# shionhonda/IaGo

Measured on AMD Instinct MI355X. Metric: self-play games/sec, higher is better.
Workload: dtype f16 MFMA operands (float32 split in 2 / 3 pieces), f32 accumulate; u64 bitboards; f32 / f64 tree statistics

## Files before the change

iago_amd/_lib.py:

```python
import ctypes as C
import os

HERE = os.path.dirname(os.path.abspath(__file__))
SO_PATH = os.environ.get("IAGO_HIP_LIB") or os.path.join(HERE, "libiago_hip.so")

IAGO_OK = 0
IAGO_ERR_INVALID, IAGO_ERR_HIP, IAGO_ERR_CAPACITY = -1, -2, -3
IAGO_MAX_TURNS = 128
IAGO_ROLLOUT_TABLE_FLOATS = 3 * 2 * 256 * 8 + 64 + 4 + 2 * 512
ROLLOUT_MODE_INDEX = 3 * 2 * 256 * 8 + 64
TRACE_PASS = 0xFF

SYMBOLS = [
    "iago_abi_version", "iago_last_error", "iago_device_count",
    "iago_legal_moves", "iago_apply_moves", "iago_play_turn", "iago_encode_planes", "iago_encode_planes_indexed",
    "iago_judge", "iago_sample_moves", "iago_augment8",
    "iago_rollout_build_table", "iago_rollout",
    "iago_policy_forward_split3", "iago_value_forward_split", "iago_value_rollout",
    "iago_mcts_reset", "iago_leaf_values", "iago_mcts_best_move", "iago_mcts_advance_root", "iago_mcts_compact",
    "iago_mcts_mix_backup_lookahead", "iago_mcts_store_priors", "iago_mcts_descend",
    "iago_mcts_search_persistent", "iago_mcts_search_capacity", "iago_mcts_search_streams_create",
    "iago_mcts_search_streams_destroy", "iago_mcts_search_split", "iago_selfplay_policy",
    "iago_policy_grad_workspace_bytes", "iago_policy_reinforce_grad", "iago_adam_chainer",
]
# ... 144 lines not shown

class MctsLookahead(C.Structure):
    _fields_ = [
        ("trigger", C.c_int32), ("slots", C.c_int32), ("next_seq", C.c_void_p), ("cache_seq", C.c_void_p),
        ("cache", C.c_void_p), ("q_count", C.c_void_p), ("q_capacity", C.c_int32), ("path_stride", C.c_int32),
        ("q_own", C.c_void_p), ("q_opp", C.c_void_p), ("q_game", C.c_void_p), ("q_seq", C.c_void_p),
        ("error", C.c_void_p), ("clear_word", C.c_void_p), ("path", C.c_void_p), ("path_len", C.c_void_p),
        ("z_log", C.c_void_p), ("z_log_n", C.c_void_p), ("z_log_rows", C.c_int32), ("reserved", C.c_int32),
        ("async_", C.c_void_p), ("value_ahead", C.c_void_p),
    ]


class MctsValueAhead(C.Structure):
    _fields_ = [
        ("x_capacity", C.c_int32), ("row_capacity", C.c_int32), ("x_count", C.c_void_p),
        ("x_game", C.c_void_p), ("x_node", C.c_void_p), ("x_own", C.c_void_p), ("x_opp", C.c_void_p),
        ("row_count", C.c_void_p), ("row_own", C.c_void_p), ("row_opp", C.c_void_p), ("row_node", C.c_void_p),
        ("row_v", C.c_void_p), ("total", C.c_void_p),
    ]


SEARCH_QUEUE_ENTRIES = 4096
SEARCH_GAMES_PER_WORKGROUP = 32
MATCH_MCTS_COLOUR_1 = 2
MATCH_MCTS_COLOUR_2 = 3
MATCH_KEY = 0x4D415443
MATCH_SEED_XOR = MATCH_KEY << 32
EXPLORE_KEY = 0x4558504C
EXPLORE_SEED_XOR = EXPLORE_KEY << 32
CAP_KEY = 0x43415050
CAP_SEED_XOR = CAP_KEY << 32
CTL_BAD_DRAW = 13
REC_DRAWN = 2
REC_FAST = 4


class MctsSearchArgs(C.Structure):
    _fields_ = [
        ("tree", C.c_void_p), ("root_own", C.c_void_p), ("root_opp", C.c_void_p), ("active", C.c_void_p),
        ("c_puct", C.c_float), ("lmbda", C.c_float), ("n_thr", C.c_int32), ("n_sims", C.c_int32),
        ("net_workgroups", C.c_int32), ("time_limit_ms", C.c_int32),
        ("value", C.c_void_p), ("policy", C.c_void_p), ("rollout", C.c_void_p),
        ("cur_node", C.c_void_p), ("cur_own", C.c_void_p), ("cur_opp", C.c_void_p), ("path", C.c_void_p),
        ("path_stride", C.c_int32), ("z_log_rows", C.c_int32), ("done", C.c_void_p), ("roll", C.c_void_p),
        ("leaf_value", C.c_void_p), ("z_log", C.c_void_p), ("z_log_n", C.c_void_p), ("q_slots", C.c_void_p),
        ("ctl", C.c_void_p), ("rep_v", C.c_void_p), ("rep_p", C.c_void_p), ("totals", C.c_void_p),
# ... 203 lines not shown
```

iago_amd/csrc/search_kernel.hip:

```cpp
#include "mcts_dev.hpp"
#include "conv_trunk_body.hpp"
#include "conv_policy_body.hpp"
#include "sample_dev.hpp"
#include "../../include/iago_hip_serving.h"

#include <cstdlib>
#include <string>
#include <vector>

namespace {
using namespace iago;
using namespace iago_mcts;

typedef unsigned long long u64;
#define RLX_AGENT __ATOMIC_RELAXED, __HIP_MEMORY_SCOPE_AGENT

constexpr uint32_t QCAP = IAGO_SEARCH_QUEUE_ENTRIES;
constexpr int CTL_FINISHED = 2, CTL_ABORT = 3;
__host__ __device__ constexpr int ctl_head(uint32_t q) { return 8 + 2 * (int)q; }
__host__ __device__ constexpr int ctl_tail(uint32_t q) { return 9 + 2 * (int)q; }
enum { ST_READY = 0, ST_WAIT_PRIOR, ST_PRIOR_READY, ST_ROLL, ST_ROLL_FRESH, ST_WAIT_VALUE, ST_HAVE_VALUE, ST_DONE, ST_TURN, ST_MOVE,
       ST_WAIT_DRAW, ST_DRAW,
       ST_IDLE };
constexpr int CTL_NO_CHILDREN = 4;
// ... 43 lines not shown
    int8_t *rec_move;
    int32_t *rec_pi;
    int32_t games_total, stream;
    u64 *vtable;
    uint32_t vtable_mask;
    int64_t *trace;
    int32_t trace_rows;
    int32_t policy_xcds;
    int32_t pair_backlog;
    int32_t pace_margin, pace_backlog;
    int32_t ahead_idle;
    int32_t roll_defer;
    int32_t path_lds_cap;
    int32_t wave;
    float vloss;
    int64_t n_slots;
    int64_t *wave_timing;
    int32_t park_empties;
    uint8_t *parked;
    int32_t *park_stones;
    uint8_t *park_pass;
    int32_t explore_turns;
    int32_t cap_fast, cap_full_256;
};

__device__ __forceinline__ u64 ld(const u64 *p) { return __hip_atomic_load(p, RLX_AGENT); }
__device__ __forceinline__ void st(u64 *p, u64 x) { __hip_atomic_store(p, x, RLX_AGENT); }

__device__ __forceinline__ void send_request(const SearchParams &S, uint32_t kind, int64_t g, uint32_t reply_tag,
                                             uint64_t own, uint64_t opp)
{
    const uint32_t t = __hip_atomic_fetch_add(&S.ctl[ctl_tail(kind)], 1u, RLX_AGENT);
    u64 *e = S.q_slots + ((u64)kind * QCAP + t % QCAP) * 8u;
    const u64 tag = (u64)(t + 1u) << 32;
    st(e + 1, tag | reply_tag);
    st(e + 2, tag | (uint32_t)own);
    st(e + 3, tag | (uint32_t)(own >> 32));
    st(e + 4, tag | (uint32_t)opp);
    st(e + 5, tag | (uint32_t)(opp >> 32));
    st(e + 0, tag | (kind << 31) | (uint32_t)g);
    atomicAdd((unsigned long long *)&S.totals[(uint32_t)g == NOBODY ? 11 : kind], 1ull);
}

__device__ __forceinline__ uint32_t vtable_slot(const SearchParams &S, uint64_t own, uint64_t opp)
{
    uint64_t h = own * 0x9E3779B97F4A7C15ull ^ (opp + 0xD1B54A32D192ED03ull) * 0xBF58476D1CE4E5B9ull;
// ... 128 lines not shown
struct Game {
    int state;
    uint32_t epoch;
    int n_done, turn, stones;
    bool pass_flg, g_over;
    uint64_t g_own, g_opp;
};

struct Cursor {
    int node, fc, k, nv, nvv;
    uint32_t vbits;
    uint64_t own, opp;
    int path_n, leaf;
    bool may_expand, leaf_fresh;
    float v_reply;
};

struct GameLds {
    uint64_t h_own[GAMES_PER_WG], h_opp[GAMES_PER_WG];
    int32_t h_stream[GAMES_PER_WG];
    int32_t h_game[GAMES_PER_WG];
    int32_t h_budget[GAMES_PER_WG];
    uint8_t h_fast[GAMES_PER_WG];
    uint32_t wg_count[6];
    int32_t roll_list[GAMES_PER_WG];
    uint32_t roll_wave[BLOCK / 64], roll_wave_old[BLOCK / 64];
    int32_t pace[4];
    uint32_t claimed;
    int8_t h_z[GAMES_PER_WG];
};
template <bool WAVE> struct GameShared : GameLds {};
template <> struct GameShared<true> : GameLds {
    int32_t wv_next[GAMES_PER_WG], wv_size[GAMES_PER_WG], wv_block[GAMES_PER_WG];
    long long wv_time[4];
};

template <bool WAVE>
__device__ __forceinline__ Slot make_slot(const SearchParams &S, const int wg)
{
    Slot I;
    I.wg = wg;
    I.tid = threadIdx.x;
    I.gl = I.tid >> 3;
    I.L = make_lane8(threadIdx.x);
    I.r = I.L.l8;
    I.mine = I.tid < 8 * S.games_per_wg;
    I.g = (int64_t)wg * S.games_per_wg + I.gl;
// ... 157 lines not shown
        }
        G.state = ST_DONE;
        if (S.trace && I.r == 0u && I.g < S.trace_rows) {
            int64_t *row = S.trace + 4 * ((int64_t)S.trace_rows - 1 - I.g);
            row[0] = wall_clock64() - t0;
            row[1] = G.epoch;
            row[2] = G.turn;
        }
    } else {
        G.state = ST_TURN;
    }
}

template <bool PARK>
__device__ __forceinline__ void turn_boundary(const SearchParams &S, const iago_row::HwParams &R, const Slot &I, GameLds &sh,
                                              Game &G, const Cursor &C, bool &busy, const long long t0)
{
    const Tree &T = S.T;
    for (int rep = 0; rep < 6; rep++) {
        const bool at_move = G.state == ST_MOVE, at_turn = G.state == ST_TURN, at_draw = G.state == ST_DRAW;
        if (__builtin_amdgcn_ballot_w64(at_move || at_turn || at_draw) == 0ull)
            break;
        busy = busy || at_move || at_turn || at_draw;
        const bool explores = S.explore_turns > 0 && at_move && G.turn < S.explore_turns;
        const bool caps = S.cap_fast > 0 && at_turn;
        uint32_t w = 0u;
        if (__builtin_amdgcn_ballot_w64(explores || caps) != 0ull)
            w = turn_word(R.key0, R.key1 ^ (caps ? CAP_KEY : EXPLORE_KEY), R.id_base + (uint32_t)sh.h_game[I.gl], (uint32_t)G.turn);
        if (caps) {
            const bool fast = cap_fast_turn(w, (uint32_t)S.cap_full_256);
            sh.h_budget[I.gl] = fast ? S.cap_fast : S.n_sims;
            sh.h_fast[I.gl] = fast ? 1 : 0;
        }
        const uint64_t lg = group8_legal(to_lane(G.g_own, I.L), to_lane(G.g_opp, I.L), I.L);
        const bool can_move = lg != 0ull && !G.g_over;
        const int code = (at_turn && can_move && !S.stream) ? (int)S.active[I.g] : 0;
        const bool match = code == 2 || code == 3;
        const bool forced = match && G.stones > 62 && __popcll(lg) == 1;
        const bool policy_turn = match && !forced && (G.turn & 1) == (code == 2 ? 1 : 0);
        if (policy_turn) {
            G.epoch++;
            if (I.r == 0u)
                send_request(S, KIND_POLICY, I.g, G.epoch, G.g_own, G.g_opp);
            G.state = ST_WAIT_DRAW;
        }
        bool park = false;
// ... 54 lines not shown
        send_request(S, KIND_POLICY, I.g, G.epoch, C.own, C.opp);
    G.state = ST_WAIT_PRIOR;
    if (sh.pace[3] > 0 && I.need_v) {
        uint64_t rest = group8_legal(to_lane(C.own, I.L), to_lane(C.opp, I.L), I.L);
        while (rest) {
            const int a2 = (int)__builtin_ctzll(rest);
            rest &= rest - 1ull;
            uint64_t c_own = C.own, c_opp = C.opp;
            place_stone(c_own, c_opp, a2, I.L);
            uint32_t known = 0u, by = 0u;
            if (I.r == 0u && !vtable_get(S, c_own, c_opp, known, by) && atomicSub(&sh.pace[3], 1) > 0)
                send_request(S, KIND_VALUE, (int64_t)NOBODY, (uint32_t)I.g, c_own, c_opp);
        }
    }
}

template <bool WAVE>
__device__ __forceinline__ void reach_leaf(const SearchParams &S, const Slot &I, GameShared<WAVE> &sh, Game &G, Cursor &C,
                                           bool descending)
{
    if (descending && C.fc >= 0 && I.r == 0u)
        S.T.overflow[I.gt] = 1;
    C.leaf = C.node;
    const float c = __uint_as_float(C.vbits);
    C.leaf_fresh = I.need_v && c != c;
    bool ask = C.leaf_fresh;
    if (S.vtable_mask) {
        uint32_t hit = 0u, bits = 0u, by = 0u;
        if (C.leaf_fresh && I.r == 0u && vtable_get(S, C.own, C.opp, bits, by)) {
            hit = 1u;
            atomicAdd((unsigned long long *)&S.totals[8], 1ull);
            if (by == (uint32_t)I.g)
                atomicAdd((unsigned long long *)&S.totals[12], 1ull);
        }
        hit = group8_add(hit);
        bits = group8_add(I.r == 0u ? bits : 0u);
        if (hit) {
            C.vbits = bits;
            ask = false;
        }
    }
    if (ask)
        G.epoch++;
    if (I.r == 0u) {
        S.cur_node[I.g] = C.node;
        S.cur_own[I.g] = C.own;
// ... 26 lines not shown
    if (grow) {
        const int kn = lg ? __popcll(lg) : 1;
        if (lg != 0ull && kn > 1 && !have_priors) {
            need_prior = true;
            descending = false;
        } else {
            C.may_expand = false;
            const uint32_t fc1 = alloc_children(T, I.gt, kn, I.r == 0u);
            if (fc1 != 0u) {
                const int nf = (int)fc1 - 1;
                make_children(T, I.base, nf, C.node, lg, I.r,
                              [&](int a) { return __uint_as_float((uint32_t)ld(&S.rep_p[I.g * 64 + a])); });
                if (I.r == 0u)
                    link_children(T, I.base + C.node, nf, kn);
                C.fc = nf;
                C.k = kn;
            }
        }
    }
    __threadfence_block();
}

template <bool WAVE>
__device__ __forceinline__ void select_child(const SearchParams &S, const Slot &I, Cursor &C, bool descending)
{
    const int kk = descending ? C.k : 0;
    const double sq = sqrt((double)(WAVE ? C.nv + C.nvv : C.nv));
    double best_v = -INFINITY;
    int best_i = 0x7fffffff;
    uint32_t pl[4] = {0u, 0u, 0u, 0u};
    for (int j0 = (int)I.r; j0 < kk; j0 += 16) {
        const int j1 = j0 + 8;
        const bool two = j1 < kk;
        const int64_t c0 = I.base + C.fc + j0, c1 = two ? I.base + C.fc + j1 : c0;
        uint4 s0, l0, s1, l1;
        node_record(S.T, c0, s0, l0);
        node_record(S.T, c1, s1, l1);
        score_child<WAVE>(S.c_puct, (double)S.vloss, s0, l0, j0, sq, best_v, best_i, pl);
        if (two)
            score_child<WAVE>(S.c_puct, (double)S.vloss, s1, l1, j1, sq, best_v, best_i, pl);
    }
    argmax_step_payload<DPP_XOR1>(best_v, best_i, pl);
    argmax_step_payload<DPP_XOR2>(best_v, best_i, pl);
    argmax_step_payload<DPP_HALF_MIRROR>(best_v, best_i, pl);
    uint64_t own = C.own, opp = C.opp;
    place_stone(own, opp, descending ? (int)(int8_t)(pl[2] & 0xFFu) : -1, I.L);
    if (descending) {
        C.own = own;
        C.opp = opp;
        cursor_to<WAVE>(C, C.fc + best_i, pl[0], pl[1], pl[2], pl[2] >> 16, pl[3]);
    }
}

template <bool WAVE>
__device__ __forceinline__ bool descend(const SearchParams &S, const Slot &I, GameShared<WAVE> &sh, Game &G, Cursor &C,
                                        int pace_limit, int &st_levels, int &st_children)
{
    bool my_turn = true;
    if constexpr (WAVE)
        my_turn = I.s_in == sh.wv_next[I.tl];
    const bool fresh_start = G.state == ST_READY && (WAVE ? my_turn : G.turn * S.n_sims + G.n_done <= pace_limit);
    bool descending = fresh_start || (G.state == ST_PRIOR_READY && my_turn);
    bool have_priors = G.state == ST_PRIOR_READY;
    bool skip_record = G.state == ST_PRIOR_READY;
    bool need_prior = false;
    if (fresh_start) {
        const int root = S.T.root[I.gt];
        C.own = I.whole ? G.g_own : S.root_own[I.gt];
        C.opp = I.whole ? G.g_opp : S.root_opp[I.gt];
        uint4 s0, l0;
        node_record(S.T, I.base + root, s0, l0);
        cursor_to<WAVE>(C, root, l0.x, s0.x, l0.z, l0.w, s0.w);
        C.path_n = 0;
        C.may_expand = true;
    }
    const bool went = descending;
    for (int depth = 0; depth < MAX_DEPTH; depth++) {
        if (descending && !skip_record) {
            if (I.r == 0u) {
                if (C.path_n < S.path_stride) {
                    if (I.path_at >= 0)
                        ((int32_t *)iago_trunk::trunk_lds)[I.path_at + C.path_n] = C.node;
                    else
                        I.gpath[C.path_n] = C.node;
                }
                else
                    S.T.overflow[I.gt] = 1;
            }
            C.path_n++;
        }
        skip_record = false;
        expand(S, I, C, descending, have_priors, need_prior);
        have_priors = false;
        descending = descending && C.fc >= 0;
        if (__builtin_amdgcn_ballot_w64(descending) == 0ull)
            break;
        st_levels += descending ? 1 : 0;
        st_children += descending ? C.k : 0;
        if (__builtin_amdgcn_ballot_w64(descending && C.k != 1) == 0ull) {
            uint4 s0, l0;
            node_record(S.T, descending ? I.base + C.fc : I.base, s0, l0);
            const bool pass_child = (int)(int8_t)(l0.z & 0xFFu) < 0;
            if (__builtin_amdgcn_ballot_w64(descending && !pass_child) == 0ull) {
                if (descending) {
                    const uint64_t t = C.own;
                    C.own = C.opp;
                    C.opp = t;
                    cursor_to<WAVE>(C, C.fc, l0.x, s0.x, l0.z, l0.w, s0.w);
                }
                continue;
            }
        }
        select_child<WAVE>(S, I, C, descending);
    }
    if (went) {
        if (need_prior)
            ask_priors(S, I, sh, G, C);
        else
            reach_leaf<WAVE>(S, I, sh, G, C, descending);
    }
    if (I.exists && I.r == 0u)
        S.roll[I.g] = (I.need_z && (G.state == ST_ROLL || G.state == ST_ROLL_FRESH)) ? 1 : 0;
    return went;
}

struct CtlWords {
    uint32_t abort, idle, t0, h0, t1, h1, play, prog, next;
};
__device__ __forceinline__ CtlWords read_ctl(const SearchParams &S, int tid)
{
    CtlWords c = {0u, 0u, 0u, 0u, 0u, 0u, 0u, 0u, 0u};
    if (tid == 0) {
        if (S.stream)
            c.next = __hip_atomic_load(&S.ctl[CTL_NEXT_GAME], RLX_AGENT);
        c.abort = __hip_atomic_load(&S.ctl[CTL_ABORT], RLX_AGENT);
        c.idle = __hip_atomic_load(&S.ctl[CTL_IDLE], RLX_AGENT);
        c.t0 = __hip_atomic_load(&S.ctl[ctl_tail(0)], RLX_AGENT);
// ... 131 lines not shown
                limit = (int)(c.prog / c.play) + S.pace_margin;
        }
        sh.pace[2] = limit;
    }
    return stop != 0;
}

__device__ __forceinline__ bool stream_claim(const SearchParams &S, const Slot &I, GameLds &sh, Game &G, bool &in_play)
{
    const Tree &T = S.T;
    const int n_here = (int)min((int64_t)S.games_per_wg, I.n_slots - (int64_t)I.wg * S.games_per_wg);
    if (I.tid == 0)
        sh.claimed = __hip_atomic_fetch_add(&S.ctl[CTL_NEXT_GAME], (uint32_t)n_here, RLX_AGENT);
    __syncthreads();
    const int64_t next = T.n_games + (int64_t)sh.claimed + I.gl;
    if (I.exists && next < S.games_total) {
        start_game(G, S.game_own[next], S.game_opp[next]);
        if (I.r == 0u) {
            S.done[I.g] = 0;
            fresh_root(T, I.g, I.base);
            atomicAdd(&sh.pace[1], 1);
        }
        sh.h_game[I.gl] = (int32_t)next;
        G.state = ST_TURN;
        in_play = true;
    }
    return __syncthreads_and(!I.mine || G.state == ST_DONE) != 0;
}

template <bool WAVE>
__device__ __forceinline__ void epilogue(const SearchParams &S, const Slot &I, GameShared<WAVE> &sh, const Game &G,
                                         int st_levels, int st_children, const long long t0)
{
    if (I.exists && I.r == 0u && S.stats) {
        if (WAVE) {
            atomicAdd(&S.stats[2 * I.gt], st_levels);
            atomicAdd(&S.stats[2 * I.gt + 1], st_children);
        } else {
            S.stats[2 * I.g] += st_levels;
            S.stats[2 * I.g + 1] += st_children;
        }
    }
    if constexpr (WAVE) {
        if (I.tid < 4 && S.wave_timing)
            atomicAdd((unsigned long long *)&S.wave_timing[I.tid], (unsigned long long)sh.wv_time[I.tid]);
    }
    if (I.exists && I.r == 0u && G.state != ST_DONE && __hip_atomic_load(&S.ctl[CTL_ABORT], RLX_AGENT) != 0u) {
        S.cur_node[I.g] = (int32_t)G.epoch;
        S.leaf_value[I.g] = (float)G.state;
    }
    if (I.tid == 0) {
        atomicAdd((unsigned long long *)&S.totals[2], (unsigned long long)sh.wg_count[0]);
        atomicAdd((unsigned long long *)&S.totals[6], (unsigned long long)sh.wg_count[1]);
        atomicAdd((unsigned long long *)&S.totals[10], (unsigned long long)sh.wg_count[2]);
        atomicAdd((unsigned long long *)&S.totals[13], (unsigned long long)sh.wg_count[3]);
        atomicAdd((unsigned long long *)&S.totals[14], (unsigned long long)sh.wg_count[4]);
        atomicAdd((unsigned long long *)&S.totals[15], (unsigned long long)sh.wg_count[5]);
        atomicAdd((unsigned long long *)&S.totals[7], (unsigned long long)(wall_clock64() - t0));
        __hip_atomic_fetch_add(&S.ctl[CTL_FINISHED], 1u, RLX_AGENT);
    }
}

template <bool WAVE, bool PARK = false>
__device__ __forceinline__ void game_workgroup(const SearchParams &S, const iago_row::HwParams &R, const long long t0, const int wg)
{
    __shared__ GameShared<WAVE> sh;
    const Slot I = make_slot<WAVE>(S, wg);
    const bool first = I.exists && I.gt < S.games_total && (S.stream || S.active[I.gt] != 0);
    Game G;
    G.state = (first && S.n_sims > 0) ? (I.whole ? ST_TURN : ST_READY) : ST_DONE;
    G.epoch = 0u;
    if constexpr (WAVE) {
        const int m = S.n_sims < I.W ? S.n_sims : I.W;
        if (G.state == ST_READY && I.s_in >= m)
            G.state = ST_IDLE;
        if (I.tid < GAMES_PER_WG) {
            sh.wv_next[I.tid] = 0;
            sh.wv_size[I.tid] = m;
            sh.wv_block[I.tid] = 0;
        }
        if (I.tid < 4)
            sh.wv_time[I.tid] = 0;
    }
    if (I.exists && I.r == 0u) {
        S.done[I.g] = 0;
        S.roll[I.g] = 0;
    }
    if (I.mine) {
        sh.h_game[I.gl] = (int32_t)I.gt;
        sh.h_budget[I.gl] = S.n_sims;
        sh.h_fast[I.gl] = 0;
    }
    const bool whole_game = I.whole && I.exists && I.g < S.games_total;
    start_game(G, whole_game ? S.game_own[I.g] : 0ull, whole_game ? S.game_opp[I.g] : 0ull);
    if (whole_game && G.state == ST_DONE && I.r == 0u)
        S.n_turns[I.g] = 0;
    Cursor C = {};
    C.fc = -1;
    int st_levels = 0, st_children = 0;
    if (I.tid < 6)
        sh.wg_count[I.tid] = 0u;
    bool deferred = false;
    bool table_ready = false;
    int contrib = 0;
    bool in_play = G.state != ST_DONE;
    if (I.tid < 4)
        sh.pace[I.tid] = I.tid == 2 ? 0x7fffffff : 0;
    __syncthreads();
    if (I.mine && in_play && I.r == 0u)
        atomicAdd(&sh.pace[1], 1);
    int pace_limit = 0x7fffffff;

    for (;;) {
        const long long c_it = WAVE ? wall_clock64() : 0;
        bool busy = false;
        if (I.mine) {
            take_replies(S, R, I, sh, G, C);
            if (!WAVE && G.state == ST_HAVE_VALUE) {
                finish_playout(S, I, sh, G, C, true, C.v_reply);
                busy = true;
            }
            if (!WAVE && I.whole)
                turn_boundary<PARK>(S, R, I, sh, G, C, busy, t0);
// ... 357 lines not shown
    if (k == 0) {
        int n_cu = 0, per = 0;
        if (hipDeviceGetAttribute(&n_cu, hipDeviceAttributeMultiprocessorCount, dev) != hipSuccess ||
            hipOccupancyMaxActiveBlocksPerMultiprocessor(&per, (const void *)search_kernel, 256, (size_t)search_lds()) != hipSuccess)
            return iago_fail(IAGO_ERR_HIP, "iago_mcts_search_capacity: the device does not answer");
        if (n_cu < 1 || per < 1 || per > 255)
            return iago_fail(IAGO_ERR_CAPACITY, "iago_mcts_search_capacity: the search kernel does not fit a CU of this device");
        k = (int32_t)(n_cu << 8 | per);
        known[dev & 63].store(k, std::memory_order_release);
    }
    *cus = k >> 8;
    *workgroups_per_cu = k & 255;
    return IAGO_OK;
}

struct iago_search_streams {
    int device;
    int32_t cus, game_cus;
    hipStream_t game, net;
    hipEvent_t ready, game_done, net_done;
};

namespace {
int check_args(const iago_mcts_search_args *a, const iago_search_wave_args *wv)
{
    if (!a || !a->tree || !a->value || !a->policy || !a->rollout)
        return iago_fail(IAGO_ERR_INVALID, "iago_mcts_search_persistent: null args");
    const iago_mcts_tree *tree = a->tree;
    if (tree->n_games < 1 || tree->capacity < 1 || !tree->nodes || ((uintptr_t)tree->nodes & 31u) || !tree->n_nodes ||
        !tree->root || !tree->overflow || !tree->has_v)
        return iago_fail(IAGO_ERR_INVALID, "iago_mcts_search_persistent: bad tree (the value cache `v` is required)");
    if (tree->n_games > 0x7FFFFFF0ll)
        return iago_fail(IAGO_ERR_INVALID, "iago_mcts_search_persistent: too many games");
    if (!a->active || !a->cur_node || !a->cur_own || !a->cur_opp || !a->path ||
        a->path_stride < 8 || !a->done || !a->roll || !a->leaf_value || !a->q_slots || !a->ctl || !a->rep_v || !a->rep_p ||
        !a->totals || !a->wg_own || !a->wg_opp || ((uintptr_t)a->q_slots & 63u) || ((uintptr_t)a->rep_p & 7u) ||
        ((uintptr_t)a->rep_v & 7u) || ((uintptr_t)a->ctl & 15u))
        return iago_fail(IAGO_ERR_INVALID, "iago_mcts_search_persistent: null or misaligned state array");
    if (a->n_thr < 1 || a->n_sims < 0 || !(a->lmbda >= 0.0f && a->lmbda <= 1.0f) || a->net_workgroups < 1)
        return iago_fail(IAGO_ERR_INVALID, "iago_mcts_search_persistent: n_thr >= 1, n_sims >= 0, 0 <= lmbda <= 1, "
                                           "net_workgroups >= 1 expected");
    if (a->max_turns < 0 || (a->max_turns > 0 && (!a->game_own || !a->game_opp || !a->n_turns)) ||
        (a->max_turns > 0 && a->rec_move && (!a->rec_own || !a->rec_opp || !a->rec_valid || !a->rec_pi)))
        return iago_fail(IAGO_ERR_INVALID, "iago_mcts_search_persistent: whole games (max_turns > 0) need game_own, game_opp, "
                                           "n_turns, and all of rec_own / rec_opp / rec_valid / rec_move / rec_pi or none");
    if (a->games_total < 0 || (a->games_total > 0 && (a->max_turns == 0 || a->n_sims < 1 || a->z_log || a->z_log_rows > 0 ||
                                                      a->trace || a->trace_rows > 0)))
        return iago_fail(IAGO_ERR_INVALID, "iago_mcts_search_persistent: games_total >= 0; a stream (games_total > 0) plays "
                                           "whole games (max_turns > 0, n_sims >= 1), without z_log or trace");
    if (a->max_turns == 0 && (!a->root_own || !a->root_opp))
        return iago_fail(IAGO_ERR_INVALID, "iago_mcts_search_persistent: root_own / root_opp expected");
    if (a->z_log_rows > 0 && (!a->z_log || !a->z_log_n))
        return iago_fail(IAGO_ERR_INVALID, "iago_mcts_search_persistent: z_log needs z_log_n");
    const iago_rollout_args *ro = a->rollout;
    const int64_t n_slots = tree->n_games * (wv ? wv->width : 1);
    if (wv && n_slots > (int64_t)QCAP)
        return iago_fail(IAGO_ERR_CAPACITY, "iago_mcts_search_wave: more slots (n_games x width) than a request ring holds");
    if (ro->n != n_slots || !ro->z || !ro->table || ((uintptr_t)ro->table & 15u) || ro->log_form || ro->trace ||
        ro->uniforms || ro->throughput_hint != 0)
        return iago_fail(IAGO_ERR_INVALID, "iago_mcts_search_persistent: product-form rollout of the n games without "
                                           "trace / uniforms expected");
    const int gpw = a->games_per_workgroup;
    if (!wv && gpw > 0 && gpw != 8 && gpw != 16 && gpw != 24 && gpw != 32)
        return iago_fail(IAGO_ERR_INVALID, "iago_mcts_search_persistent: games_per_workgroup is 0 (= 32), 8, 16 or 32");
    if (a->max_cus < 0)
        return iago_fail(IAGO_ERR_INVALID, "iago_mcts_search_persistent: max_cus < 0");
    if (a->vtable_slots > 0 && (!a->vtable || ((uintptr_t)a->vtable & 31u) || (a->vtable_slots & (a->vtable_slots - 1)) != 0))
        return iago_fail(IAGO_ERR_INVALID, "iago_mcts_search_persistent: vtable must be 32-byte aligned, vtable_slots a "
                                           "power of two");
    return IAGO_OK;
}

struct SearchGrid {
    int gpw;
    int64_t n_slots, n_game_wgs, net_wgs, grid;
    int path_lds_cap, game_lds;
};

int size_grid(const iago_mcts_search_args *a, iago_search_streams *sp, const iago_search_wave_args *wv, bool park, SearchGrid &G)
{
    G.gpw = wv ? GAMES_PER_WG : a->games_per_workgroup > 0 ? a->games_per_workgroup : GAMES_PER_WG;
    G.n_slots = a->tree->n_games * (wv ? wv->width : 1);
    G.n_game_wgs = (G.n_slots + G.gpw - 1) / G.gpw;
    int32_t cus = 0, per_cu = 0;
    if (const int rc = iago_mcts_search_capacity(&cus, &per_cu))
        return rc;
    int64_t resident = (int64_t)(a->max_cus > 0 && a->max_cus < cus ? a->max_cus : cus) * per_cu;
    G.path_lds_cap = SEARCH_IMG_TOP;
    G.game_lds = 0;
    if (sp) {
        int dev = 0;
        if (hipGetDevice(&dev) != hipSuccess || dev != sp->device || sp->cus != cus)
            return iago_fail(IAGO_ERR_INVALID, "iago_mcts_search_split: the streams belong to another device");
        if (a->max_cus != 0)
            return iago_fail(IAGO_ERR_INVALID, "iago_mcts_search_split: max_cus must be 0 (the split owns the device's CUs)");
        const size_t want = (size_t)G.gpw * (size_t)a->path_stride * 4u;
        const void *game_kernel = park ? (const void *)search_game_park_kernel : (const void *)search_game_kernel;
        static std::atomic<int32_t> static_lds_of[2] = {{-1}, {-1}};
        std::atomic<int32_t> &static_lds = static_lds_of[park ? 1 : 0];
        int32_t fixed = static_lds.load(std::memory_order_acquire);
        if (fixed < 0) {
            hipFuncAttributes fa;
            if (hipFuncGetAttributes(&fa, game_kernel) != hipSuccess)
                return iago_fail(IAGO_ERR_HIP, "iago_mcts_search_split: hipFuncGetAttributes failed");
// ... 99 lines not shown
    S.wave_timing = wv ? wv->timing : nullptr;
    S.max_turns = a->max_turns;
    S.game_own = a->game_own;
    S.game_opp = a->game_opp;
    S.n_turns = a->n_turns;
    S.rec_own = a->rec_own;
    S.rec_opp = a->rec_opp;
    S.rec_valid = a->rec_valid;
    S.rec_move = a->rec_move;
    S.rec_pi = a->rec_pi;
    S.stream = a->games_total > 0 ? 1 : 0;
    S.games_total = a->games_total > 0 ? a->games_total : (int32_t)a->tree->n_games;
    S.vtable = a->vtable_slots > 0 ? (u64 *)a->vtable : nullptr;
    S.vtable_mask = a->vtable_slots > 0 ? (uint32_t)(a->vtable_slots - 1) : 0u;
    S.trace = a->trace_rows > 0 ? a->trace : nullptr;
    S.trace_rows = a->trace_rows;
    S.park_empties = -1;
    S.parked = nullptr;
    S.park_stones = nullptr;
    S.park_pass = nullptr;
    S.explore_turns = 0;
    S.cap_fast = 0;
    S.cap_full_256 = 256;
    return S;
}

int net_params(const iago_mcts_search_args *a, iago_trunk::TrunkRParams &VP, iago_policy::PolicyParams &PP, iago_row::HwParams &R)
{
    if (const int rc = iago_trunk::value_params_of(a->value, VP))
        return rc;
    VP.count_lo = 0;
    VP.count_hi = 0x7fffffff;
    if (const int rc = iago_policy::policy_params_of(a->policy, PP))
        return rc;
    R = iago_row::hw_params_of(a->rollout);
    R.own = a->cur_own;
    R.opp = a->cur_opp;
    R.mask = a->roll;
    R.stream_ids = a->done;
    return IAGO_OK;
}

int zero_polled(const iago_mcts_search_args *a, int64_t n_slots, void *stream)
{
    if (hipMemsetAsync(a->ctl, 0, 64, (hipStream_t)stream) != hipSuccess ||
        hipMemsetAsync(a->q_slots, 0, (size_t)2 * QCAP * 64, (hipStream_t)stream) != hipSuccess ||
// ... 238 lines not shown
    static std::atomic<uint64_t> configured_arena{0};
    if (iago_reserve_lds((const void *)search_arena_kernel, lds, configured_arena,
                         "iago_mcts_search_arena: cannot reserve the nets' LDS image"))
        return IAGO_ERR_HIP;
    static std::atomic<int32_t> per_known[64];
    int dev = 0;
    if (hipGetDevice(&dev) != hipSuccess)
        return iago_fail(IAGO_ERR_HIP, "iago_mcts_search_arena: hipGetDevice failed");
    int per = per_known[dev & 63].load(std::memory_order_acquire);
    if (per == 0) {
        if (hipOccupancyMaxActiveBlocksPerMultiprocessor(&per, (const void *)search_arena_kernel, 256, (size_t)lds) != hipSuccess)
            return iago_fail(IAGO_ERR_HIP, "iago_mcts_search_arena: the device does not answer");
        if (per < 1)
            return iago_fail(IAGO_ERR_CAPACITY, "iago_mcts_search_arena: the arena kernel does not fit a CU of this device");
        per_known[dev & 63].store(per, std::memory_order_release);
    }
    int64_t use_cus = cus;
    for (int i = 0; i < 2; i++)
        if (set[i]->max_cus > 0 && set[i]->max_cus < use_cus)
            use_cus = set[i]->max_cus;
    const int64_t resident = use_cus * per;
    int64_t games = 0;
    for (int i = 0; i < 2; i++) {
        G[i].gpw = set[i]->games_per_workgroup > 0 ? set[i]->games_per_workgroup : GAMES_PER_WG;
        G[i].n_slots = set[i]->tree->n_games;
        G[i].n_game_wgs = (G[i].n_slots + G[i].gpw - 1) / G[i].gpw;
        G[i].path_lds_cap = SEARCH_IMG_TOP;
        G[i].game_lds = 0;
        games += G[i].n_game_wgs;
    }
    if (games + 2 > resident)
        return iago_fail(IAGO_ERR_CAPACITY, "iago_mcts_search_arena: both agents' game workgroups and two net workgroups do "
                                            "not fit the device together (fewer games per launch, or one search after the other)");
    const int64_t net_wgs = want < resident - games ? want : resident - games;
    const int64_t grid = games + net_wgs;
    ArenaArgs args;
    ArenaSet *const P = args.set;
    for (int i = 0; i < 2; i++) {
        const iago_mcts_search_args *x = set[i];
        G[i].net_wgs = net_wgs;
        G[i].grid = grid;
        if (x->value->n < 4 * grid || x->policy->n < 4 * grid || x->value->planes || x->value->index || x->value->n_dev ||
            x->policy->index || x->policy->n_dev || !x->value->own || x->value->own != x->wg_own ||
            x->value->opp != x->wg_opp || x->policy->own != x->wg_own || x->policy->opp != x->wg_opp)
            return iago_fail(IAGO_ERR_INVALID, "iago_mcts_search_arena: each agent's nets read their rows from its wg_own / "
                                               "wg_opp (four rows per workgroup of the WHOLE grid: n >= 4 x (both agents' game "
                                               "workgroups + net workgroups)), no gather list, no device count");
// ... 100 lines not shown
```

iago_amd/engine.py:

```python
import collections
import ctypes as C
import numbers
import os

import numpy as np
import torch

from . import _lib, ops
from ._lib import MctsTree, check

START_OWN = 0x0000000810000000
START_OPP = 0x0000001008000000
HANDICAP_CELLS = (2 * 8 + 4, 3 * 8 + 5, 4 * 8 + 2, 5 * 8 + 3)
STREAM_REC_BYTES = 4 << 30


def _p(t):
    return C.c_void_p(t.data_ptr())


_stream = ops._stream

PlayRules = collections.namedtuple("PlayRules", "solve_empties explore_turns playout_cap")
NO_RULES = PlayRules(None, 0, None)
# ... 102 lines not shown
               "action": i8[:, 24].numpy(), "n_visits": rec[:, 0].numpy(), "q": f32[:, 1].numpy(),
               "p": f32[:, 2].numpy()}

        def rec(i, depth):
            d = dict(n=int(arr["n_visits"][i]), Q=float(arr["q"][i]), P=float(arr["p"][i]),
                     children={}, order=[])
            fc, k = int(arr["first_child"][i]), int(arr["n_children"][i])
            if fc >= 0:
                d["order"] = [int(arr["action"][fc + j]) for j in range(k)]
                if depth < max_depth:
                    for j in range(k):
                        d["children"][str(int(arr["action"][fc + j]))] = rec(fc + j, depth + 1)
            return d

        return rec(int(self.root[g].item()), 0)


class BatchedMCTS(object):

    def __init__(self, n_games, policy_fn, value_fn, rollout_weights, lmbda=0.5, c_puct=1.0,
                 n_thr=15, capacity=4096, seed=0, game_id_base=0, device="cuda", use_graph=False,
                 sync_free=None, lookahead=None, lookahead_slots=None, value_cache=None, lookahead_overlap=None,
                 z_log_rows=0, async_steps=None, async_parts=None, value_ahead=None, persistent=None,
                 net_workgroups=None, max_cus=None, split=None, wave=1, virtual_loss=1.0):
        if n_thr < 1:
            raise ValueError("n_thr must be >= 1")
        if isinstance(wave, bool) or wave not in (1, 8, 16, 32):
            raise ValueError("wave must be 1, 8, 16 or 32, not %r" % (wave,))
        virtual_loss = float(virtual_loss)
        if not (0.0 <= virtual_loss < float("inf")):
            raise ValueError("virtual_loss must be a finite number >= 0, not %r" % (virtual_loss,))
        self.wave, self.virtual_loss = int(wave), virtual_loss
        self.wave_entry = self.wave > 1
        ns = n_games * self.wave
        want = _split_arg(split if split is not None else os.environ.get("IAGO_SEARCH_SPLIT", "auto"))
        per_playout_asked = bool(use_graph or async_steps or value_ahead or lookahead is not None
                                 or lookahead_overlap is not None or sync_free is not None)
        self.n_games = n_games
        self.policy_fn, self.value_fn, self.rollout_weights = policy_fn, value_fn, rollout_weights
        self.lmbda, self.c_puct, self.n_thr = float(lmbda), float(c_puct), int(n_thr)
        self.seed, self.game_id_base = seed, game_id_base
        kw = dict(device=device)
        can_cache = (value_fn is not None and self.lmbda < 1.0
                     and getattr(value_fn, "forward_boards_counted", None) is not None
                     and getattr(value_fn, "split_f16", False))
        if value_cache is None:
            value_cache = can_cache
        if value_cache and not can_cache:
            raise ValueError("value_cache needs a value net with forward_boards_counted (split-f16 path) and lmbda < 1")
# ... 175 lines not shown
            self._la_stale = torch.zeros(n_games, dtype=torch.bool, **kw)
            self._la_stale_any = False

            def reset_lookahead(mask):
                if mask is None:
                    self._la_next_seq.zero_()
                    self._la_cache_seq.fill_(-1)
                    self._la_stale.zero_()
                else:
                    m = mask.bool()
                    self._la_next_seq[m] = 0
                    self._la_cache_seq[m] = -1
                    self._la_stale[m] = False
            self.tree.reset_hooks = [reset_lookahead]
        self.value_ahead = bool(getattr(self, "value_ahead", False))
        if self.persistent:
            if net_workgroups is None:
                net_workgroups = int(os.environ.get("IAGO_PERSISTENT_NET", "0")) or max(32, 8 * n_games)
            self.net_workgroups = max(1, min(int(net_workgroups), self.resident_workgroups - n_gw))
            if self.split_cus:
                self.net_workgroups = max(1, min(int(net_workgroups), self.resident_workgroups
                                                 - max(self.split_cus, self.resident_workgroups // 8)))
            grid = n_gw + self.net_workgroups
            self.PATH_STRIDE = 520
            i64 = torch.int64
            self._ps = dict(
                path=torch.zeros((ns, self.PATH_STRIDE), dtype=torch.int32, **kw),
                done=torch.zeros(ns, dtype=torch.int32, **kw), roll=torch.zeros(ns, dtype=torch.uint8, **kw),
                q_slots=torch.zeros(2 * _lib.SEARCH_QUEUE_ENTRIES * 8, dtype=i64, **kw), ctl=torch.zeros(16, dtype=torch.int32, **kw),
                rep_v=torch.zeros(ns, dtype=i64, **kw), rep_p=torch.zeros(ns * 64, dtype=i64, **kw),
                totals=torch.zeros(16, dtype=i64, **kw), wg_own=torch.zeros(4 * grid, dtype=i64, **kw),
                wg_opp=torch.zeros(4 * grid, dtype=i64, **kw), wg_v=torch.zeros(4 * grid, dtype=torch.float32, **kw),
                wg_probs=torch.zeros((4 * grid, 64), dtype=torch.float32, **kw))
            slots = int(os.environ.get("IAGO_PERSISTENT_TABLE", str(1 << 20)))
            self._vtable = torch.zeros(4 * slots, dtype=i64, **kw) if slots > 0 else None
            self.z_log = torch.zeros((z_log_rows, n_games), dtype=torch.int8, **kw) if z_log_rows else None
            self.z_log_n = torch.zeros(n_games, dtype=torch.int32, **kw) if z_log_rows else None
            self.time_limit_ms = int(os.environ.get("IAGO_PERSISTENT_LIMIT_MS", "4000"))
            self.wave_timing = torch.zeros(4, dtype=i64, **kw)
            self._wave_active = None
        self.tree.reset_hooks = list(getattr(self.tree, "reset_hooks", ())) + [
            lambda mask: setattr(self, "_live_after_compaction", 0)]
        can_async = bool(self.lookahead and self.value_cache and getattr(self, "fused_descent", False)
                         and getattr(self, "_la_path", None) is not None and self.fused_leaf_eval
                         and 0.0 < self.lmbda < 1.0 and rollout_weights is not None and not rollout_weights.log_form
                         and getattr(value_fn, "forward_boards_async", None) is not None)
        if async_steps is None:
            async_steps = can_async and os.environ.get("IAGO_ASYNC", "0") == "1"
        if async_steps and not can_async:
            raise ValueError("async_steps needs the look-ahead playout with the value cache, the one-launch descent, "
                             "the path backup, the fused leaf evaluation (0 < lmbda < 1, product-form rollout "
                             "weights) and a value net with forward_boards_async")
        self.async_steps = bool(async_steps)
        self.n_steps = 0
# ... 576 lines not shown
            check(_lib.lib().iago_mcts_search_persistent(C.byref(a), _stream()), "iago_mcts_search_persistent")
        if ev is not None:
            e1.record()
            ev.append((e0, e1))
        self._ps_keep = keep + (park,)

    def _search_args(self, own, opp, active, n_sims, game=None):
        if self.rollout_hook is not None:
            raise ValueError("rollout_hook is not available in the persistent search (z_log_rows records the z)")
        ps = self._ps
        sid = self.sim_counter - (1 << 32) if self.sim_counter >= (1 << 31) else self.sim_counter
        ro = ops.rollout_prepare(self.cur_own, self.cur_opp, self.rollout_weights, seed=self.seed,
                                 id_base=self.game_id_base, stream_id=sid, out=self._rollout_out)
        with torch.no_grad():
            va, keep_v = self.value_fn.search_args(ps["wg_own"], ps["wg_opp"], ps["wg_v"])
            pa, keep_p = self.policy_fn.search_args(ps["wg_own"], ps["wg_opp"], ps["wg_probs"])
        a = _lib.MctsSearchArgs()
        a.tree = C.addressof(self.tree.c)
        if own is not None:
            a.root_own, a.root_opp = own.data_ptr(), opp.data_ptr()
        a.active = active.data_ptr()
        a.c_puct, a.lmbda, a.n_thr, a.n_sims = self.c_puct, self.lmbda, self.n_thr, int(n_sims)
        a.net_workgroups, a.time_limit_ms = self.net_workgroups, self.time_limit_ms
        a.games_per_workgroup = self.games_per_workgroup
        a.pace_margin = self.pace_margin
        a.max_cus = self.max_cus
        a.value, a.policy, a.rollout = C.addressof(va), C.addressof(pa), C.addressof(ro.args)
        a.cur_node, a.cur_own, a.cur_opp = self.cur_node.data_ptr(), self.cur_own.data_ptr(), self.cur_opp.data_ptr()
        a.path, a.path_stride = ps["path"].data_ptr(), self.PATH_STRIDE
        a.done, a.roll, a.leaf_value = ps["done"].data_ptr(), ps["roll"].data_ptr(), self.leaf_value.data_ptr()
        if self.z_log is not None:
            a.z_log, a.z_log_n, a.z_log_rows = self.z_log.data_ptr(), self.z_log_n.data_ptr(), self.z_log.shape[0]
        a.q_slots, a.ctl = ps["q_slots"].data_ptr(), ps["ctl"].data_ptr()
        a.rep_v, a.rep_p, a.totals = ps["rep_v"].data_ptr(), ps["rep_p"].data_ptr(), ps["totals"].data_ptr()
        a.stats = self.stats.data_ptr() if self.stats is not None else None
        a.wg_own, a.wg_opp = ps["wg_own"].data_ptr(), ps["wg_opp"].data_ptr()
        if game is not None:
            a.max_turns = int(game["max_turns"])
            a.time_limit_ms = max(self.time_limit_ms, int(os.environ.get("IAGO_PERSISTENT_GAME_LIMIT_MS", "60000")))
            a.games_total = int(game.get("games_total", 0))
            if a.games_total:
                a.time_limit_ms = min(a.time_limit_ms * -(-a.games_total // self.n_games), 0x7FFFFFFF)
            a.game_own, a.game_opp, a.n_turns = game["own"].data_ptr(), game["opp"].data_ptr(), game["n_turns"].data_ptr()
            a.rec_own, a.rec_opp = game["rec_own"].data_ptr(), game["rec_opp"].data_ptr()
            a.rec_valid, a.rec_move, a.rec_pi = (game["rec_valid"].data_ptr(), game["rec_move"].data_ptr(),
                                                 game["rec_pi"].data_ptr())
        if self._vtable is not None:
# ... 811 lines not shown
```

include/iago_hip.h:

```cpp
#ifndef IAGO_HIP_H
#define IAGO_HIP_H

#include <stdint.h>

#if defined(__GNUC__)
#define IAGO_API __attribute__((visibility("default")))
#else
#define IAGO_API
#endif

#ifdef __cplusplus
extern "C" {
#endif

typedef enum iago_status {
    IAGO_OK = 0,
    IAGO_ERR_INVALID = -1,
    IAGO_ERR_HIP = -2,
    IAGO_ERR_CAPACITY = -3
} iago_status;

#define IAGO_PASS (-1)
#define IAGO_TRACE_PASS 0xFF
#define IAGO_MAX_TURNS 128
// ... 31 lines not shown

typedef struct iago_rollout_args {
    const uint64_t *own;
    const uint64_t *opp;
    int64_t n;
    const float *table;
    const float *uniforms;
    uint64_t seed;
    uint32_t id_base;
    uint32_t stream_id;
    const uint32_t *stream_id_dev;
    int8_t *z;
    uint64_t *final_own;
    uint64_t *final_opp;
    uint8_t *n_turns;
    uint8_t *trace;
    int log_form;
    int throughput_hint;
} iago_rollout_args;

IAGO_API int iago_rollout(const iago_rollout_args *args, void *stream);



typedef struct iago_policy_split3_args {
    const uint64_t *own, *opp;
    const int64_t *index;
    const int32_t *n_dev;
    int64_t n;
    const float *w1, *b1;
    const void *w_hi[7], *w_mid[7], *w_lo[7];
    const float *bias[7];
    const float *w9, *b10;
    float *probs;
    uint32_t *overflow;
    int32_t parts;
    int32_t scratch_rows;
    void *scratch;
} iago_policy_split3_args;
IAGO_API int iago_policy_forward_split3(const iago_policy_split3_args *args, void *stream);
typedef struct iago_value_split_args {
    const float *planes;
    const uint64_t *own, *opp;
    int64_t n;
    const float *w1, *b1;
    const void *w_hi[7], *w_lo[7];
    const float *bias[7];
// ... 26 lines not shown
typedef struct iago_mcts_tree {
    int64_t n_games;
    int32_t capacity;
    int32_t has_v;
    iago_mcts_node *nodes;
    int32_t *n_nodes;
    int32_t *root;
    int32_t *overflow;
} iago_mcts_tree;

IAGO_API int iago_mcts_reset(const iago_mcts_tree *tree, const uint8_t *mask, void *stream);

IAGO_API int iago_leaf_values(const float *v, const int8_t *z, float lmbda, float *leaf_value,
                              int64_t n, void *stream);

IAGO_API int iago_mcts_best_move(const iago_mcts_tree *tree, const uint8_t *active, int8_t *move,
                                 int32_t *visits, void *stream);

IAGO_API int iago_mcts_advance_root(const iago_mcts_tree *tree, const uint8_t *mask,
                                    const int8_t *move, void *stream);

IAGO_API int iago_mcts_compact(const iago_mcts_tree *tree, const iago_mcts_tree *scratch, int32_t *order,
                               const uint8_t *mask, void *stream);



struct iago_mcts_async;
struct iago_mcts_value_ahead;
typedef struct iago_mcts_lookahead {
    int32_t trigger, slots;
    int32_t *next_seq;
    int32_t *cache_seq;
    float *cache;
    int32_t *q_count;
    int32_t q_capacity;
    int32_t path_stride;
    uint64_t *q_own, *q_opp;
    int32_t *q_game, *q_seq;
    int32_t *error;
    int32_t *clear_word;
    int32_t *path;
    int32_t *path_len;
    int8_t *z_log;
    int32_t *z_log_n;
    int32_t z_log_rows;
    int32_t reserved;
    const struct iago_mcts_async *async;
    const struct iago_mcts_value_ahead *value_ahead;
} iago_mcts_lookahead;
IAGO_API int iago_mcts_mix_backup_lookahead(const iago_mcts_tree *tree, const uint8_t *active,
                                            const int32_t *cur_node, const uint64_t *cur_own,
                                            const uint64_t *cur_opp, const float *v, const int8_t *z, float lmbda,
                                            float *leaf_value, uint32_t *counter,
                                            const iago_mcts_lookahead *la, void *stream);
IAGO_API int iago_mcts_store_priors(const iago_mcts_lookahead *la, const float *probs, int64_t *total,
                                    void *stream);

IAGO_API int iago_mcts_descend(const iago_mcts_tree *tree, const uint64_t *root_own, const uint64_t *root_opp,
                               const uint8_t *active, float c_puct, int32_t n_thr, int32_t *cur_node,
                               uint64_t *cur_own, uint64_t *cur_opp, uint64_t *legal, int32_t *stats,
                               const iago_mcts_lookahead *la, int64_t *fresh_index, int32_t *fresh_count,
                               int64_t *fresh_total, void *stream);


#define IAGO_SEARCH_QUEUE_ENTRIES 4096
#define IAGO_SEARCH_GAMES_PER_WORKGROUP 32
typedef struct iago_mcts_search_args {
    const iago_mcts_tree *tree;
    const uint64_t *root_own, *root_opp;
    const uint8_t *active;
    float c_puct, lmbda;
    int32_t n_thr, n_sims;
    int32_t net_workgroups, time_limit_ms;
    const iago_value_split_args *value;
    const iago_policy_split3_args *policy;
    const iago_rollout_args *rollout;
    int32_t *cur_node;
    uint64_t *cur_own, *cur_opp;
    int32_t *path;
    int32_t path_stride, z_log_rows;
    int32_t *done;
    uint8_t *roll;
    float *leaf_value;
    int8_t *z_log;
    int32_t *z_log_n;
    void *q_slots;
    uint32_t *ctl;
    void *rep_v, *rep_p;
    int64_t *totals;
// ... 76 lines not shown
```

Before: 3006.

## Skip re-descending forced single-child chains by jumping to the last recorded path node

Adds a chain-skip mode to the persistent MCTS search kernel. For each game it records in LDS where the last non-trivial branching point on the previous path was. On the next descent, once the cursor reaches that node it jumps directly to the recorded leaf, swapping colours for odd skip lengths, instead of re-running select_child through a chain of single-child or pass nodes. The flag is carried in a spare bit of games_per_workgroup and is enabled by default from Python. This adds LDS state and branching, and correctness depends on the skipped nodes being forced moves whose statistics need no per-level update.

```diff
diff --git a/iago_amd/_lib.py b/iago_amd/_lib.py
--- a/iago_amd/_lib.py
+++ b/iago_amd/_lib.py
@@ -190,6 +190,7 @@
 
 SEARCH_QUEUE_ENTRIES = 4096
 SEARCH_GAMES_PER_WORKGROUP = 32
+SEARCH_CHAIN_SKIP = 0x100
 MATCH_MCTS_COLOUR_1 = 2
 MATCH_MCTS_COLOUR_2 = 3
 MATCH_KEY = 0x4D415443
diff --git a/iago_amd/csrc/search_kernel.hip b/iago_amd/csrc/search_kernel.hip
--- a/iago_amd/csrc/search_kernel.hip
+++ b/iago_amd/csrc/search_kernel.hip
@@ -89,6 +89,7 @@
     uint8_t *park_pass;
     int32_t explore_turns;
     int32_t cap_fast, cap_full_256;
+    int32_t chain_skip;
 };
 
 __device__ __forceinline__ u64 ld(const u64 *p) { return __hip_atomic_load(p, RLX_AGENT); }
@@ -263,7 +264,8 @@
     int32_t h_game[GAMES_PER_WG];
     int32_t h_budget[GAMES_PER_WG];
     uint8_t h_fast[GAMES_PER_WG];
-    uint32_t wg_count[6];
+    uint32_t wg_count[7];
+    int32_t ch_from[GAMES_PER_WG], ch_len[GAMES_PER_WG], ch_run[GAMES_PER_WG];
     int32_t roll_list[GAMES_PER_WG];
     uint32_t roll_wave[BLOCK / 64], roll_wave_old[BLOCK / 64];
     int32_t pace[4];
@@ -467,6 +469,8 @@
         if (__builtin_amdgcn_ballot_w64(at_move || at_turn || at_draw) == 0ull)
             break;
         busy = busy || at_move || at_turn || at_draw;
+        if (at_move || at_turn || at_draw)
+            sh.ch_from[I.gl] = -1;
         const bool explores = S.explore_turns > 0 && at_move && G.turn < S.explore_turns;
         const bool caps = S.cap_fast > 0 && at_turn;
         uint32_t w = 0u;
@@ -567,6 +571,13 @@
     if (descending && C.fc >= 0 && I.r == 0u)
         S.T.overflow[I.gt] = 1;
     C.leaf = C.node;
+    if constexpr (!WAVE) {
+        if (S.chain_skip && I.r == 0u) {
+            const int run = sh.ch_run[I.gl];
+            sh.ch_from[I.gl] = (!descending && C.path_n <= S.path_stride && run < C.path_n - 1) ? run : -1;
+            sh.ch_len[I.gl] = C.path_n;
+        }
+    }
     const float c = __uint_as_float(C.vbits);
     C.leaf_fresh = I.need_v && c != c;
     bool ask = C.leaf_fresh;
@@ -639,7 +650,7 @@
 }
 
 template <bool WAVE>
-__device__ __forceinline__ void select_child(const SearchParams &S, const Slot &I, Cursor &C, bool descending)
+__device__ __forceinline__ int select_child(const SearchParams &S, const Slot &I, Cursor &C, bool descending)
 {
     const int kk = descending ? C.k : 0;
     const double sq = sqrt((double)(WAVE ? C.nv + C.nvv : C.nv));
@@ -661,12 +672,14 @@
     argmax_step_payload<DPP_XOR2>(best_v, best_i, pl);
     argmax_step_payload<DPP_HALF_MIRROR>(best_v, best_i, pl);
     uint64_t own = C.own, opp = C.opp;
-    place_stone(own, opp, descending ? (int)(int8_t)(pl[2] & 0xFFu) : -1, I.L);
+    const int action = descending ? (int)(int8_t)(pl[2] & 0xFFu) : -1;
+    place_stone(own, opp, action, I.L);
     if (descending) {
         C.own = own;
         C.opp = opp;
         cursor_to<WAVE>(C, C.fc + best_i, pl[0], pl[1], pl[2], pl[2] >> 16, pl[3]);
     }
+    return action;
 }
 
 template <bool WAVE>
@@ -691,8 +704,44 @@
         C.path_n = 0;
         C.may_expand = true;
     }
+    int jump_at = -1, jumped = 0;
+    if constexpr (!WAVE) {
+        if (S.chain_skip) {
+            jump_at = descending ? sh.ch_from[I.gl] : -1;
+            if (fresh_start && I.r == 0u)
+                sh.ch_run[I.gl] = 0;
+        }
+    }
     const bool went = descending;
     for (int depth = 0; depth < MAX_DEPTH; depth++) {
+        if constexpr (!WAVE) {
+            if (descending && depth + jumped >= MAX_DEPTH) {
+                descending = false;
+                jumped = -1;
+            }
+            if (descending && !skip_record && C.path_n == jump_at) {
+                const int len = sh.ch_len[I.gl], n_skip = len - 1 - jump_at;
+                const int last = path_entry(I.path_at, I.gpath, len - 1);
+                if (path_entry(I.path_at, I.gpath, jump_at) == C.node && depth + n_skip < MAX_DEPTH) {
+                    uint4 s0, l0;
+                    node_record(S.T, I.base + last, s0, l0);
+                    if (n_skip & 1) {
+                        const uint64_t t = C.own;
+                        C.own = C.opp;
+                        C.opp = t;
+                    }
+                    cursor_to<WAVE>(C, last, l0.x, s0.x, l0.z, l0.w, s0.w);
+                    C.path_n = len;
+                    skip_record = true;
+                    jumped = n_skip;
+                    st_levels += n_skip;
+                    st_children += n_skip;
+                    if (I.r == 0u)
+                        atomicAdd(&sh.wg_count[6], (uint32_t)n_skip);
+                }
+                jump_at = -1;
+            }
+        }
         if (descending && !skip_record) {
             if (I.r == 0u) {
                 if (C.path_n < S.path_stride) {
@@ -728,8 +777,15 @@
                 continue;
             }
         }
-        select_child<WAVE>(S, I, C, descending);
-    }
+        const bool one = C.k == 1;
+        const int action = select_child<WAVE>(S, I, C, descending);
+        if constexpr (!WAVE) {
+            if (S.chain_skip && descending && I.r == 0u && !(one && action < 0))
+                sh.ch_run[I.gl] = C.path_n;
+        }
+    }
+    if constexpr (!WAVE)
+        descending = descending || jumped < 0;
     if (went) {
         if (need_prior)
             ask_priors(S, I, sh, G, C);
@@ -907,6 +963,7 @@
             atomicAdd(&sh.pace[1], 1);
         }
         sh.h_game[I.gl] = (int32_t)next;
+        sh.ch_from[I.gl] = -1;
         G.state = ST_TURN;
         in_play = true;
     }
@@ -941,6 +998,8 @@
         atomicAdd((unsigned long long *)&S.totals[13], (unsigned long long)sh.wg_count[3]);
         atomicAdd((unsigned long long *)&S.totals[14], (unsigned long long)sh.wg_count[4]);
         atomicAdd((unsigned long long *)&S.totals[15], (unsigned long long)sh.wg_count[5]);
+        if (S.chain_skip)
+            atomicAdd((unsigned long long *)&S.totals[16], (unsigned long long)sh.wg_count[6]);
         atomicAdd((unsigned long long *)&S.totals[7], (unsigned long long)(wall_clock64() - t0));
         __hip_atomic_fetch_add(&S.ctl[CTL_FINISHED], 1u, RLX_AGENT);
     }
@@ -975,6 +1034,7 @@
         sh.h_game[I.gl] = (int32_t)I.gt;
         sh.h_budget[I.gl] = S.n_sims;
         sh.h_fast[I.gl] = 0;
+        sh.ch_from[I.gl] = -1;
     }
     const bool whole_game = I.whole && I.exists && I.g < S.games_total;
     start_game(G, whole_game ? S.game_own[I.g] : 0ull, whole_game ? S.game_opp[I.g] : 0ull);
@@ -983,7 +1043,7 @@
     Cursor C = {};
     C.fc = -1;
     int st_levels = 0, st_children = 0;
-    if (I.tid < 6)
+    if (I.tid < 7)
         sh.wg_count[I.tid] = 0u;
     bool deferred = false;
     bool table_ready = false;
@@ -1387,6 +1447,11 @@
 };
 
 namespace {
+int games_per_wg_of(const iago_mcts_search_args *a)
+{
+    return a->games_per_workgroup > 0 ? (a->games_per_workgroup & ~IAGO_SEARCH_CHAIN_SKIP) : a->games_per_workgroup;
+}
+
 int check_args(const iago_mcts_search_args *a, const iago_search_wave_args *wv)
 {
     if (!a || !a->tree || !a->value || !a->policy || !a->rollout)
@@ -1425,7 +1490,7 @@
         ro->uniforms || ro->throughput_hint != 0)
         return iago_fail(IAGO_ERR_INVALID, "iago_mcts_search_persistent: product-form rollout of the n games without "
                                            "trace / uniforms expected");
-    const int gpw = a->games_per_workgroup;
+    const int gpw = games_per_wg_of(a);
     if (!wv && gpw > 0 && gpw != 8 && gpw != 16 && gpw != 24 && gpw != 32)
         return iago_fail(IAGO_ERR_INVALID, "iago_mcts_search_persistent: games_per_workgroup is 0 (= 32), 8, 16 or 32");
     if (a->max_cus < 0)
@@ -1444,7 +1509,7 @@
 
 int size_grid(const iago_mcts_search_args *a, iago_search_streams *sp, const iago_search_wave_args *wv, bool park, SearchGrid &G)
 {
-    G.gpw = wv ? GAMES_PER_WG : a->games_per_workgroup > 0 ? a->games_per_workgroup : GAMES_PER_WG;
+    G.gpw = wv ? GAMES_PER_WG : games_per_wg_of(a) > 0 ? games_per_wg_of(a) : GAMES_PER_WG;
     G.n_slots = a->tree->n_games * (wv ? wv->width : 1);
     G.n_game_wgs = (G.n_slots + G.gpw - 1) / G.gpw;
     int32_t cus = 0, per_cu = 0;
@@ -1590,6 +1655,7 @@
     S.explore_turns = 0;
     S.cap_fast = 0;
     S.cap_full_256 = 256;
+    S.chain_skip = (!wv && a->games_per_workgroup > 0 && (a->games_per_workgroup & IAGO_SEARCH_CHAIN_SKIP)) ? 1 : 0;
     return S;
 }
 
@@ -1874,7 +1940,7 @@
     const int64_t resident = use_cus * per;
     int64_t games = 0;
     for (int i = 0; i < 2; i++) {
-        G[i].gpw = set[i]->games_per_workgroup > 0 ? set[i]->games_per_workgroup : GAMES_PER_WG;
+        G[i].gpw = games_per_wg_of(set[i]) > 0 ? games_per_wg_of(set[i]) : GAMES_PER_WG;
         G[i].n_slots = set[i]->tree->n_games;
         G[i].n_game_wgs = (G[i].n_slots + G[i].gpw - 1) / G[i].gpw;
         G[i].path_lds_cap = SEARCH_IMG_TOP;
diff --git a/iago_amd/engine.py b/iago_amd/engine.py
--- a/iago_amd/engine.py
+++ b/iago_amd/engine.py
@@ -148,9 +148,13 @@
                  n_thr=15, capacity=4096, seed=0, game_id_base=0, device="cuda", use_graph=False,
                  sync_free=None, lookahead=None, lookahead_slots=None, value_cache=None, lookahead_overlap=None,
                  z_log_rows=0, async_steps=None, async_parts=None, value_ahead=None, persistent=None,
-                 net_workgroups=None, max_cus=None, split=None, wave=1, virtual_loss=1.0):
+                 net_workgroups=None, max_cus=None, split=None, wave=1, virtual_loss=1.0, chain_skip=True,
+                 path_stride=None):
         if n_thr < 1:
             raise ValueError("n_thr must be >= 1")
+        if path_stride is not None and (isinstance(path_stride, bool) or int(path_stride) != path_stride or path_stride < 8):
+            raise ValueError("path_stride must be None or an int >= 8, not %r" % (path_stride,))
+        self.chain_skip = bool(chain_skip)
         if isinstance(wave, bool) or wave not in (1, 8, 16, 32):
             raise ValueError("wave must be 1, 8, 16 or 32, not %r" % (wave,))
         virtual_loss = float(virtual_loss)
@@ -372,14 +376,14 @@
                 self.net_workgroups = max(1, min(int(net_workgroups), self.resident_workgroups
                                                  - max(self.split_cus, self.resident_workgroups // 8)))
             grid = n_gw + self.net_workgroups
-            self.PATH_STRIDE = 520
+            self.PATH_STRIDE = 520 if path_stride is None else int(path_stride)
             i64 = torch.int64
             self._ps = dict(
                 path=torch.zeros((ns, self.PATH_STRIDE), dtype=torch.int32, **kw),
                 done=torch.zeros(ns, dtype=torch.int32, **kw), roll=torch.zeros(ns, dtype=torch.uint8, **kw),
                 q_slots=torch.zeros(2 * _lib.SEARCH_QUEUE_ENTRIES * 8, dtype=i64, **kw), ctl=torch.zeros(16, dtype=torch.int32, **kw),
                 rep_v=torch.zeros(ns, dtype=i64, **kw), rep_p=torch.zeros(ns * 64, dtype=i64, **kw),
-                totals=torch.zeros(16, dtype=i64, **kw), wg_own=torch.zeros(4 * grid, dtype=i64, **kw),
+                totals=torch.zeros(17, dtype=i64, **kw), wg_own=torch.zeros(4 * grid, dtype=i64, **kw),
                 wg_opp=torch.zeros(4 * grid, dtype=i64, **kw), wg_v=torch.zeros(4 * grid, dtype=torch.float32, **kw),
                 wg_probs=torch.zeros((4 * grid, 64), dtype=torch.float32, **kw))
             slots = int(os.environ.get("IAGO_PERSISTENT_TABLE", str(1 << 20)))
@@ -1002,7 +1006,7 @@
         a.active = active.data_ptr()
         a.c_puct, a.lmbda, a.n_thr, a.n_sims = self.c_puct, self.lmbda, self.n_thr, int(n_sims)
         a.net_workgroups, a.time_limit_ms = self.net_workgroups, self.time_limit_ms
-        a.games_per_workgroup = self.games_per_workgroup
+        a.games_per_workgroup = self.games_per_workgroup | (_lib.SEARCH_CHAIN_SKIP if self.chain_skip else 0)
         a.pace_margin = self.pace_margin
         a.max_cus = self.max_cus
         a.value, a.policy, a.rollout = C.addressof(va), C.addressof(pa), C.addressof(ro.args)
diff --git a/include/iago_hip.h b/include/iago_hip.h
--- a/include/iago_hip.h
+++ b/include/iago_hip.h
@@ -77,7 +77,6 @@
 IAGO_API int iago_rollout(const iago_rollout_args *args, void *stream);
 
 
-
 typedef struct iago_policy_split3_args {
     const uint64_t *own, *opp;
     const int64_t *index;
@@ -150,7 +149,6 @@
 
 IAGO_API int iago_mcts_compact(const iago_mcts_tree *tree, const iago_mcts_tree *scratch, int32_t *order,
                                const uint8_t *mask, void *stream);
-
 
 
 struct iago_mcts_async;
@@ -190,9 +188,9 @@
                                const iago_mcts_lookahead *la, int64_t *fresh_index, int32_t *fresh_count,
                                int64_t *fresh_total, void *stream);
 
-
 #define IAGO_SEARCH_QUEUE_ENTRIES 4096
 #define IAGO_SEARCH_GAMES_PER_WORKGROUP 32
+#define IAGO_SEARCH_CHAIN_SKIP 0x100
 typedef struct iago_mcts_search_args {
     const iago_mcts_tree *tree;
     const uint64_t *root_own, *root_opp;
```

Measured after the change: 3042, median of 6. 1.2% higher.
